# arghyasur1991/Spark-TTS

Hardware: AMD Instinct MI355X
Metric: audio samples/sec (whole node), Spark-TTS-0.5B greedy (higher is better)
Workload: dtype bf16 weights + KV, fp32 activations/accumulate (LLM); vocoder: fp32 operands split into 2 bf16 planes, 3 products on the bf16 matrix pipe, fp32 accumulate

## Files before the change

### spark-tts_amd/csrc/smi_llm.hip

```cpp
#include "smi_common.h"
#include <stdio.h>
#include <string.h>
#include <cmath>
#include <map>
#include <mutex>
#include <vector>

namespace {

constexpr int kMaxRows = SMI_MAX_ROWS;
constexpr int kHeadDim = 64;

struct RowDesc {
  int32_t slot, pos, token, flags;
};

struct SampRec {
  int32_t mode;
  int32_t top_k;
  float inv_temp, top_p;
  unsigned long long seed;
  int32_t has_seed, pad;
};

// ... 3247 lines not shown
  uint8_t slot_feat[kMaxRows];
  int lm_restrict;
  int seq_dirty[kMaxRows];
  SeqRec* seq;
  std::vector<SeqRec> hseq;
  int* tlist;
  std::vector<int32_t> host_tlist;
  float* lp;
  float* lp_part; float2* lp_rowc;
  uint16_t* phist;
  int64_t* poll_dev; int64_t* poll_host;
  int32_t* pen_idx; size_t pen_idx_cap;
  std::vector<int32_t> host_pen_idx;
  float* logits; int* tok;
  float* cand_v; int* cand_i; unsigned int* cand_n;
  unsigned long long* stamps; int stamps_on;
  int max_steps;
  int tune[4];
  int graph_steps;
  int pf_inline;
  int pf_qkv_eighths;
  int prefetch_mask, prefetch_rows;
  int tune2;
  int pgemm_min_rows;
  int pg_min[4];
  int wd_parts;
  int exact;
  int gu1_lo;
  int gu1_rows;
  hipGraphExec_t graph; uint64_t graph_id;
  std::map<hipGraphExec_t, hipStream_t> graph_last;
  std::map<uint64_t, hipGraphExec_t> graph_cache;
  hipEvent_t ev0, ev1;
  std::vector<RowDesc> host_rows;
#ifdef SMI_DIAG
  EngState eng;
  int eng_on;
#endif
};

namespace {

std::vector<const void*>& lds_big_kernels() {
  static std::vector<const void*> v;
  return v;
}
bool lds_big_register(const void* f) {
  lds_big_kernels().push_back(f);
  return true;
}
template <auto F>
struct LdsBig {
  static inline const bool reg = lds_big_register((const void*)F);
};
constexpr int kLdsBigBytes = 160 * 1024;

void pages_release(smi_llm* L, int slot) {
  for (int i = 0; i < L->slot_pages[slot]; ++i) {
    const int32_t pg = L->hptab[(size_t)slot * L->ppslot + i];
    if (--L->page_ref[pg] == 0) L->free_pages.push_back(pg);
  }
  L->slot_pages[slot] = 0;
}
void pages_share(smi_llm* L, int src, int dst, int n) {
  for (int i = 0; i < n; ++i) {
    const int32_t pg = L->hptab[(size_t)src * L->ppslot + i];
// ... 664 lines not shown

template <int PRO, int EPI, int NTW = 2, int WR = 1, int RING = 0, int XMAP = 0, int TWO = 0, int MTB = 8>
int launch_pgemm(const smi_llm* L, GemmP p, hipStream_t st, int nsplit = 1) {
  constexpr int cols = (4 / WR) * NTW;
  constexpr int rows = MTB * 16;
  const dim3 grid2((p.NT + cols - 1) / cols, (p.M + rows - 1) / rows);
  dim3 grid = XMAP ? dim3(grid2.x * grid2.y) : grid2;
  constexpr size_t lds = (RING ? (size_t)RING * (12 * rows + cols * 64) : (size_t)2 * 12 * rows) * 16 + (TWO ? 0 : rows * 4);
  if constexpr (lds > 64 * 1024) {
    static_cast<void>(LdsBig<k_pgemm<PRO, EPI, 1, NTW, WR, RING, XMAP, TWO, MTB>>::reg);
    static_cast<void>(LdsBig<k_pgemm<PRO, EPI, 0, NTW, WR, RING, XMAP, TWO, MTB>>::reg);
    static_assert(lds <= (size_t)kLdsBigBytes, "k_pgemm: LDS beyond the opted-in window");
  }
  const int mtiles = (p.M + 15) / 16;
  if (nsplit > 1) {
    SMI_REQUIRE(EPI == EPI_RESID && XMAP && RING >= 3 && p.kseg > 0 && nsplit <= 16, "launch_pgemm: split-K is the RESID ring form's");
    SMI_REQUIRE(L->pslab && (size_t)nsplit * p.NT * mtiles * 1024 <= L->pslab_bytes, "launch_pgemm: partial slab too small");
    p.slab = L->pslab; p.slab_mt = mtiles;
    grid = dim3(grid2.x * grid2.y, nsplit);
  }
  if (L->cfg.kv_dtype) hipLaunchKernelGGL((k_pgemm<PRO, EPI, 1, NTW, WR, RING, XMAP, TWO, MTB>), grid, dim3(256), lds, st, p);
  else hipLaunchKernelGGL((k_pgemm<PRO, EPI, 0, NTW, WR, RING, XMAP, TWO, MTB>), grid, dim3(256), lds, st, p);
  SMI_LAUNCH_CHECK();
  if (nsplit > 1) {
    DownCP d;
    d.W = nullptr; d.NT = p.NT; d.KT = p.KT; d.M = p.M; d.wperm = 0; d.XS = nullptr; d.part = L->pslab;
    d.Y = p.Y; d.Yin = p.Yin; d.gamma_next = p.gamma_next; d.XSout = p.XSout; d.ssout = p.ssout;
    hipLaunchKernelGGL((k_resid_comb<1, 1>), dim3(p.NT * mtiles), dim3(64), 0, st, d, nsplit, mtiles);
    SMI_LAUNCH_CHECK();
  }
  return SMI_OK;
}

int launch_layers_big(smi_llm* L, const RowDesc* rows, int M, int family, hipStream_t st) {
  const smi_llm_cfg& c = L->cfg;
  const bool pg = family == PF_PGEMM;
  const bool gq = L->pg_forced ? M < L->pg_min[0] : !pg, go = L->pg_forced ? M < L->pg_min[1] : !pg,
             gg = L->pg_forced ? M < L->pg_min[2] : !pg, gd = L->pg_forced ? M < L->pg_min[3] : !pg;
  const int np_from_d = gd ? L->NTh * 4 : L->NTh, np_from_o = go ? L->NTh * 4 : L->NTh;
  const bool few = M <= L->pg_split_rows && !(L->tune2 & 16384);
  const int kseg_o = (L->KTq + kPgSegO - 1) / kPgSegO, kseg_d = (L->KTi + kPgSegD - 1) / kPgSegD;
  const int nseg_o = (L->KTq + kseg_o - 1) / kseg_o, nseg_d = (L->KTi + kseg_d - 1) / kseg_d;
  int rc;
  for (int l = 0; l < c.num_layers; ++l) {
    const GemmP p = gemm_operands(L, KQKV, l, L->big, rows, M, np_from_d);
    if (gq) rc = launch_gemm<1, 16, 2, 1, PRO_NORM, EPI_QKV>(L, p, st);
    else if (L->tune2 & 16384) rc = launch_pgemm<PRO_NORM, EPI_QKV>(L, p, st);
    else if (few) rc = launch_pgemm<PRO_NORM, EPI_QKV, 2, 2, 6, 1, 0, 4>(L, p, st);
    else rc = launch_pgemm<PRO_NORM, EPI_QKV, 6, 2, 3, 1>(L, p, st);
    if (rc) return rc;
    if (l == c.num_layers - 1) break;
    const AttnP a = attn_operands(L, l, L->big, rows, M);
    if (L->tune2 & 1024) {
      if ((rc = c.kv_dtype ? launch_attn<1>(L, a, 0, st) : launch_attn<0>(L, a, 0, st))) return rc;
    } else {
      const dim3 ag((unsigned)((M + kAttnWaves - 1) / kAttnWaves), (unsigned)c.num_heads);
      if (!c.kv_dtype && L->attn_pf2 && L->pf_ntiles > 0 && c.head_dim == 64) {
        const int tasks = L->pf_ntiles * c.num_heads;
        hipLaunchKernelGGL(k_attn_pf2, dim3((tasks + 3) / 4), dim3(256), 0, st, a, (const PfTile*)L->pf_tiles, L->pf_ntiles);
      } else if (c.kv_dtype) hipLaunchKernelGGL((k_attn_pf<1>), ag, dim3(kAttnWaves * 64), 0, st, a);
      else hipLaunchKernelGGL((k_attn_pf<0>), ag, dim3(kAttnWaves * 64), 0, st, a);
      SMI_LAUNCH_CHECK();
    }
    GemmP o = gemm_operands(L, KO, l, L->big, rows, M, np_from_d);
    o.kseg = kseg_o;
    if (go) rc = launch_oproj(L, o, M, st);
    else if (L->tune2 & 16384) rc = launch_pgemm<PRO_PLAIN, EPI_RESID>(L, o, st);
    else if (few) rc = launch_pgemm<PRO_PLAIN, EPI_RESID, 2, 2, 6, 1, 0, 4>(L, o, st, nseg_o);
    else rc = launch_pgemm<PRO_PLAIN, EPI_RESID, 4, 2, 4, 1>(L, o, st);
    if (rc) return rc;
    const GemmP g = gemm_operands(L, KGU, l, L->big, rows, M, np_from_o);
    if (gg) rc = launch_gemm<1, 8, 4, 1, PRO_NORM, EPI_SWIGLU, 1, 2>(L, g, st);
    else if (L->tune2 & 512) rc = launch_pgemm<PRO_NORM, EPI_SWIGLU>(L, g, st);
    else if (L->tune2 & 16384) rc = launch_pgemm<PRO_NORM, EPI_SWIGLU, 4>(L, g, st);
    else if (L->tune2 & 32768) rc = launch_pgemm<PRO_NORM, EPI_SWIGLU, 8, 2, 3>(L, g, st);
    else if (few) rc = launch_pgemm<PRO_NORM, EPI_SWIGLU, 2, 2, 4, 0, 0, 4>(L, g, st);
    else rc = launch_pgemm<PRO_NORM, EPI_SWIGLU, 8, 2, 2, 0, 1>(L, g, st);
    if (rc) return rc;
    GemmP d = gemm_operands(L, KD, l, L->big, rows, M, np_from_o);
    d.wperm = L->wd_parts; d.kseg = kseg_d;
    if (gd) rc = launch_gemm<1, 16, 2, 5, PRO_PLAIN, EPI_RESID>(L, d, st);
    else if (L->tune2 & 16384) rc = launch_pgemm<PRO_PLAIN, EPI_RESID>(L, d, st);
    else if (few) rc = launch_pgemm<PRO_PLAIN, EPI_RESID, 2, 2, 6, 1, 0, 4>(L, d, st, nseg_d);
// ... 11 lines not shown
void work_free(Work& w) {
  void* ptrs[] = {w.h, w.q, w.xs_h, w.xs_attn, w.xs_act, w.ss};
  for (void* q : ptrs)
    if (q) (void)hipFree(q);
  w = Work{};
}

int ensure_big(smi_llm* L, int rows) {
  if (rows <= L->big_rows) return SMI_OK;
  work_free(L->big);
  L->big_rows = 0;
  if (L->pslab) (void)hipFree(L->pslab);
  L->pslab = nullptr; L->pslab_bytes = 0;
  {
    const size_t mt = ((size_t)(rows < kPgSplitRows ? rows : kPgSplitRows) + 15) / 16;
    const size_t bytes = (size_t)16 * L->NTh * mt * 1024;
    if (hipMalloc((void**)&L->pslab, bytes) != hipSuccess) { smi_set_error("hipMalloc(prefill split-K slab, %zu bytes) failed", bytes); return SMI_ENOMEM; }
    L->pslab_bytes = bytes;
  }
  if (!work_alloc(L, L->big, (size_t)rows)) { smi_set_error("hipMalloc(prefill workspace for %d rows) failed", rows); return SMI_ENOMEM; }
  L->big_rows = rows;
  return SMI_OK;
}

int launch_embed(smi_llm* L, const RowDesc* rows, int M, hipStream_t st) {
  hipLaunchKernelGGL(k_embed, dim3((M + 3) / 4), dim3(256), 0, st, (const uint16_t*)sec(L, SMI_LLM_LM_HEAD, 0), L->KTh, rows, M,
                     (const float*)sec(L, SMI_LLM_LN1, 0), L->dec.h, L->dec.xs_h, L->dec.ss, L->NTh * 4, L->exact);
  SMI_LAUNCH_CHECK();
  return SMI_OK;
}

int launch_layers(smi_llm* L, const RowDesc* rows, int M, bool kv_only_last, hipStream_t st) {
  int rc;
  for (int l = 0; l < L->cfg.num_layers; ++l) {
    if ((rc = launch_one(L, KQKV, l, rows, M, nullptr, st))) return rc;
    if (kv_only_last && l == L->cfg.num_layers - 1) break;
    if ((rc = launch_one(L, KATTN, l, rows, M, nullptr, st))) return rc;
    if ((rc = launch_one(L, KO, l, rows, M, nullptr, st))) return rc;
    if ((rc = launch_one(L, KGU, l, rows, M, nullptr, st))) return rc;
    if ((rc = launch_one(L, KD, l, rows, M, nullptr, st))) return rc;
  }
  return SMI_OK;
}

int launch_step(smi_llm* L, int M, hipStream_t st) {
  int rc;
  if (eng_usable(L, L->rows, M)) {
    if ((rc = eng_launch(L, st))) return rc;
  } else if ((rc = launch_layers(L, L->rows, M, false, st))) return rc;
  if ((rc = launch_one(L, KLM, 0, L->rows, M, nullptr, st))) return rc;
  return launch_one(L, KFIN, 0, L->rows, M, nullptr, st);
}

int ensure_plan(smi_llm* L, size_t rows) {
  if (rows <= L->plan_cap) return SMI_OK;
  if (L->plan) (void)hipFree(L->plan);
  L->plan = nullptr; L->plan_cap = 0;
  size_t cap = rows + 1024;
  if (hipMalloc((void**)&L->plan, cap * sizeof(RowDesc)) != hipSuccess) {
    smi_set_error("hipMalloc(prefill plan, %zu rows) failed", cap);
    return SMI_ENOMEM;
  }
  L->plan_cap = cap;
  return SMI_OK;
}

struct PollArgs {
  int32_t slot[kMaxRows];
  int32_t from[kMaxRows];
};
__global__ __launch_bounds__(64) void k_poll(const int64_t* hist, const int32_t* count, const int32_t* finished, int max_steps,
                                             PollArgs a, int cap, int64_t* stage) {
  const int i = blockIdx.x, sl = a.slot[i], from = a.from[i];
  int64_t* rec = stage + (size_t)i * (1 + cap);
  const int cnt = count[sl];
  if (threadIdx.x == 0) {
    int2 head; head.x = cnt; head.y = finished[sl];
    *(int2*)rec = head;
  }
  int end = cnt < max_steps ? cnt : max_steps;
  if (end - from > cap) end = from + cap;
  for (int t = from + (int)threadIdx.x; t < end; t += 64) rec[1 + (t - from)] = hist[(size_t)t * kMaxRows + sl];
}

// ... 171 lines not shown
      hipMemset(L->count, 0, kMaxRows * 4) != hipSuccess || hipMemset(L->finished, 0, kMaxRows * 4) != hipSuccess ||
      hipMemset(L->step, 0, 4) != hipSuccess) {
    smi_set_error("hipMemset of scratch failed");
    smi_llm_destroy(L);
    return SMI_EHIP;
  }
  if (hipFuncSetAttribute((const void*)k_lm32<7>, hipFuncAttributeMaxDynamicSharedMemorySize, 160 * 1024) != hipSuccess) (void)hipGetLastError();
  if (hipFuncSetAttribute((const void*)k_lm32<8>, hipFuncAttributeMaxDynamicSharedMemorySize, 160 * 1024) != hipSuccess) (void)hipGetLastError();
  if (hipFuncSetAttribute((const void*)k_lm32<7, 1>, hipFuncAttributeMaxDynamicSharedMemorySize, 160 * 1024) != hipSuccess) (void)hipGetLastError();
  if (hipFuncSetAttribute((const void*)k_lm32<8, 1>, hipFuncAttributeMaxDynamicSharedMemorySize, 160 * 1024) != hipSuccess) (void)hipGetLastError();
  {
    static std::mutex mu;
    static bool done[64] = {};
    int dev = 0;
    std::lock_guard<std::mutex> lk(mu);
    if (hipGetDevice(&dev) != hipSuccess || dev < 0 || dev >= 64) {
      smi_set_error("smi_llm_create: no current device");
      smi_llm_destroy(L);
      return SMI_EHIP;
    }
    for (size_t i = 0; i < lds_big_kernels().size() && !done[dev]; ++i)
      if (hipFuncSetAttribute(lds_big_kernels()[i], hipFuncAttributeMaxDynamicSharedMemorySize, kLdsBigBytes) != hipSuccess) {
        smi_set_error("smi_llm_create: hipFuncSetAttribute(MaxDynamicSharedMemorySize) failed: %s", hipGetErrorString(hipGetLastError()));
        smi_llm_destroy(L);
        return SMI_EHIP;
      }
    done[dev] = true;
  }
  if (hipEventCreate(&L->ev0) != hipSuccess || hipEventCreate(&L->ev1) != hipSuccess) {
    smi_set_error("hipEventCreate failed");
    smi_llm_destroy(L);
    return SMI_EHIP;
  }
#ifdef SMI_DIAG
  L->eng_on = 0;
  snprintf(L->eng.why, sizeof(L->eng.why), "off (opt-in: SPARKMI_ENGINE=1 or smi_llm_set_engine)");
  { const char* e = smi_env("SPARKMI_ENGINE");
    if (e && e[0] == '1') {
      const int rce = eng_create(L);
      if (rce) { smi_llm_destroy(L); return rce; }
      L->eng_on = L->eng.enabled;
    }
  }
#endif
  *out = L;
  return SMI_OK;
}

int smi_llm_destroy(smi_llm* L) {
  if (!L) return SMI_OK;
  graphs_flush(L);
  eng_destroy(L);
  work_free(L->dec);
  work_free(L->big);
  void* ptrs[] = {L->part_o, L->h2, L->dpart, L->fuse_cnt, L->rows, L->plan, L->pf_tiles, L->pval, L->pidx, L->hist,
                  L->count, L->finished, L->step, L->ctl, L->ptab, L->kcache, L->vcache, L->logits, L->tok, L->cand_v, L->cand_i, L->cand_n, L->stamps, L->pslab, L->apart,
                  L->phist, L->pen_idx, L->lp, L->lp_part, L->lp_rowc, L->tlist, L->poll_dev, L->seq};
  for (void* q : ptrs)
    if (q) (void)hipFree(q);
  if (L->poll_host) (void)hipHostFree(L->poll_host);
  if (L->ev0) (void)hipEventDestroy(L->ev0);
  if (L->ev1) (void)hipEventDestroy(L->ev1);
  delete L;
  return SMI_OK;
}

int smi_llm_set_sampling(smi_llm* L, int do_sample, float temperature, int top_k, float top_p, uint64_t seed) {
  SMI_REQUIRE(L, "smi_llm_set_sampling: null handle");
  if (do_sample) {
    SMI_REQUIRE(temperature > 0.f, "smi_llm_set_sampling: temperature must be > 0");
    SMI_REQUIRE(top_k >= 1 && top_k <= kSampleCap, "smi_llm_set_sampling: top_k must be in 1..%d", kSampleCap);
    SMI_REQUIRE(top_p > 0.f && top_p <= 1.f, "smi_llm_set_sampling: top_p must be in (0, 1]");
    if (top_k > L->cfg.vocab_size) top_k = L->cfg.vocab_size;
  }
  const bool changed = L->do_sample != (do_sample ? 1 : 0) ||
                       (do_sample && (L->temperature != temperature || L->top_k != top_k || L->top_p != top_p));
  L->do_sample = do_sample ? 1 : 0;
  L->temperature = temperature; L->top_k = top_k; L->top_p = top_p; L->seed = seed;
  L->hctl.seed = seed;
  SMI_HIP(hipMemcpy(&L->ctl->seed, &seed, sizeof(seed), hipMemcpyHostToDevice));
  if (changed) graphs_flush(L);
  return SMI_OK;
}

static int validate_prompts(const smi_llm* L, const int64_t* ids, const int32_t* lens, int B, int P_max) {
  for (int b = 0; b < B; ++b) {
    SMI_REQUIRE(lens[b] >= 1 && lens[b] <= P_max, "smi_llm_prefill: lens[%d]=%d outside 1..%d", b, lens[b], P_max);
    SMI_REQUIRE(lens[b] < L->cfg.max_positions, "smi_llm_prefill: prompt %d longer than max_positions", b);
    for (int t = 0; t < lens[b]; ++t) {
      const int64_t id = ids[(size_t)b * P_max + t];
      SMI_REQUIRE(id >= 0 && id < L->cfg.vocab_size, "smi_llm_prefill: token id %lld out of range", (long long)id);
    }
  }
  return SMI_OK;
}

static int prefill_prompts(smi_llm* L, const int64_t* ids, const int32_t* lens, int B, int P_max, const int32_t* slots,
                           size_t* tail_off, hipStream_t st, const int32_t* n_ret = nullptr, const int32_t* tail_slots = nullptr,
                           const std::vector<RowDesc>* extra = nullptr) {
  size_t total = 0;
  { const int rcv = validate_prompts(L, ids, lens, B, P_max); if (rcv) return rcv; }
  for (int b = 0; b < B; ++b) total += lens[b] - 1;
  {
    int longest = 0;
    for (int b = 0; b < B; ++b) longest = lens[b] > longest ? lens[b] : longest;
    L->attn_seg = segs_for(longest);
  }
  const bool chunks_only = smi_env("SPARKMI_PREFILL_CHUNKS") != nullptr || L->exact;
  auto cls_of = [&](int b) -> int {
    const int r = lens[b] - 1;
    if (chunks_only) return 0;
    if (L->pg_forced) return total > (size_t)kMaxRows ? 3 : 0;
    return r <= kMaxRows ? 0 : r < L->pf_long ? 1 : 2;
  };
  size_t ncls[4] = {0, 0, 0, 0};
  for (int b = 0; b < B; ++b) ncls[cls_of(b)] += lens[b] - 1;
  const size_t nchunks = (ncls[0] + kMaxRows - 1) / kMaxRows;
  const size_t off2 = 0, off1 = ncls[2], off3 = off1 + ncls[1], off0 = off3 + ncls[3], tail = off0 + nchunks * kMaxRows;
  int rc;
  const size_t nextra = extra ? extra->size() : 0;
  if ((rc = ensure_plan(L, tail + kMaxRows + nextra))) return rc;
  L->host_rows.assign(tail + kMaxRows + nextra, RowDesc{0, 0, 0, 0});
  {
    size_t w[4] = {off0, off1, off2, off3};
    for (int b = 0; b < B; ++b) {
      size_t& r = w[cls_of(b)];
      for (int t = 0; t + 1 < lens[b]; ++t) L->host_rows[r++] = RowDesc{slots[b], t, (int32_t)ids[(size_t)b * P_max + t], 0};
    }
  }
  for (int b = 0, j = 0; b < B; ++b)
    for (int r = 0; r < (n_ret ? n_ret[b] : 1); ++r, ++j)
      L->host_rows[tail + j] = RowDesc{tail_slots ? tail_slots[j] : slots[b], lens[b] - 1, (int32_t)ids[(size_t)b * P_max + lens[b] - 1], 0};
  for (size_t e = 0; e < nextra; ++e) L->host_rows[tail + kMaxRows + e] = (*extra)[e];
  SMI_HIP(hipMemcpyAsync(L->plan, L->host_rows.data(), L->host_rows.size() * sizeof(RowDesc), hipMemcpyHostToDevice, st));
  const size_t pass_off[3] = {off2, off1, off3}, pass_rows[3] = {ncls[2], ncls[1], ncls[3]};
  const int pass_family[3] = {PF_PGEMM, PF_GROUPED, PF_PGEMM};
  for (int ps = 0; ps < 3; ++ps) {
    if (pass_rows[ps] == 0) continue;
    constexpr size_t kBigRows = 4096;
    if ((rc = ensure_big(L, (int)(pass_rows[ps] < kBigRows ? pass_rows[ps] : kBigRows)))) return rc;
    for (size_t q0 = 0; q0 < pass_rows[ps]; q0 += kBigRows) {
      const size_t r0 = pass_off[ps] + q0;
      const int M = (int)((pass_rows[ps] - q0) < kBigRows ? (pass_rows[ps] - q0) : kBigRows);
      const RowDesc* rows = L->plan + r0;
      L->pf_ntiles = 0;
      if (!L->cfg.kv_dtype && L->attn_pf2) {
        std::vector<PfTile>& T = L->host_tiles;
        T.clear();
        for (int i = 0; i < M;) {
          const RowDesc& a0 = L->host_rows[r0 + i];
          int n = 1;
          while (n < 16 && i + n < M && L->host_rows[r0 + i + n].slot == a0.slot && L->host_rows[r0 + i + n].pos == a0.pos + n) ++n;
          T.push_back(PfTile{i, n, a0.slot, a0.pos});
          i += n;
        }
        if (T.size() > L->pf_tiles_cap) {
          if (L->pf_tiles) (void)hipFree(L->pf_tiles);
          L->pf_tiles = nullptr; L->pf_tiles_cap = 0;
          const size_t cap = T.size() + 256;
          if (hipMalloc((void**)&L->pf_tiles, cap * sizeof(PfTile)) != hipSuccess) { smi_set_error("hipMalloc(prefill attention tiles) failed"); return SMI_ENOMEM; }
          L->pf_tiles_cap = cap;
        }
        SMI_HIP(hipMemcpyAsync(L->pf_tiles, T.data(), T.size() * sizeof(PfTile), hipMemcpyHostToDevice, st));
        L->pf_ntiles = (int)T.size();
      }
      const bool d_grouped = L->pg_forced ? M < L->pg_min[3] : pass_family[ps] == PF_GROUPED;
      hipLaunchKernelGGL(k_embed, dim3((M + 3) / 4), dim3(256), 0, st, (const uint16_t*)sec(L, SMI_LLM_LM_HEAD, 0), L->KTh, rows, M,
                         (const float*)sec(L, SMI_LLM_LN1, 0), L->big.h, L->big.xs_h, L->big.ss, d_grouped ? L->NTh * 4 : L->NTh, 0);
      SMI_LAUNCH_CHECK();
      if ((rc = launch_layers_big(L, rows, M, pass_family[ps], st))) return rc;
    }
  }
  for (size_t c = 0; c < nchunks; ++c) {
    const int M = (int)((ncls[0] - c * kMaxRows) < (size_t)kMaxRows ? (ncls[0] - c * kMaxRows) : kMaxRows);
    const RowDesc* rows = L->plan + off0 + c * kMaxRows;
    if ((rc = launch_embed(L, rows, M, st))) return rc;
    if ((rc = launch_layers(L, rows, M, true, st))) return rc;
  }
  *tail_off = tail;
  return SMI_OK;
}

static void live_set(smi_llm* L, const int* slots, int n) {
  L->B = n;
  L->live_order.assign(slots, slots + n);
  L->identity_slots = 1;
  L->lm_restrict = n > 0;
  for (int b = 0; b < n; ++b) {
    L->identity_slots &= slots[b] == b;
    L->lm_restrict &= (L->slot_feat[slots[b]] & F_ALLOW) != 0;
  }
  L->graph = nullptr;
}

static int validate_eos(const int64_t* eos_ids, int n_eos) {
  SMI_REQUIRE(n_eos >= 0 && n_eos <= SMI_MAX_EOS && (n_eos == 0 || eos_ids), "eos list: 0..%d ids", SMI_MAX_EOS);
  return SMI_OK;
}

static int gen_reset(smi_llm* L, const int64_t* eos_ids, int n_eos, int nseq, hipStream_t st) {
  L->started = 0;
  for (int b = 0; b < kMaxRows; ++b) L->hctl.seqid[b] = nseq ? b : 0;
  slots_clear(L);
  L->admit_seq = nseq;
  if (L->paged)
    for (int b = 0; b < kMaxRows; ++b) pages_release(L, b);
  memset(L->slot_busy, 0, sizeof(L->slot_busy));
  memset(L->slot_len, 0, sizeof(L->slot_len));
  live_set(L, nullptr, 0);
  for (int e = 0; e < SMI_MAX_EOS; ++e) L->hctl.eos[e] = e < n_eos ? (long long)eos_ids[e] : -1;
  L->hctl.n_eos = n_eos;
  L->hctl.seed = L->seed;
  SMI_HIP(hipMemcpyAsync(L->ctl, &L->hctl, sizeof(Ctl), hipMemcpyHostToDevice, st));
  SMI_HIP(hipMemsetAsync(L->count, 0, kMaxRows * 4, st));
  SMI_HIP(hipMemsetAsync(L->finished, 0, kMaxRows * 4, st));
  SMI_HIP(hipMemsetAsync(L->step, 0, 4, st));
  L->session = nseq == 0;
  L->started = 1;
  return SMI_OK;
}

int smi_llm_prefill(smi_llm* L, const int64_t* ids, const int32_t* lens, int B, int P_max, const int64_t* eos_ids, int n_eos,
                    void* stream) {
  SMI_REQUIRE(L && ids && lens, "smi_llm_prefill: null argument");
  SMI_REQUIRE(B >= 1 && B <= L->cfg.max_slots, "smi_llm_prefill: B=%d outside 1..%d", B, L->cfg.max_slots);
  hipStream_t st = (hipStream_t)stream;
  int32_t slots[kMaxRows];
  for (int b = 0; b < kMaxRows; ++b) slots[b] = b;
  int rc;
  if ((rc = validate_prompts(L, ids, lens, B, P_max)) || (rc = validate_eos(eos_ids, n_eos))) return rc;
  if (L->paged) {
    long need = 0;
    for (int b = 0; b < B; ++b) need += (lens[b] + (1 << L->pshift) - 1) >> L->pshift;
    if (need > L->cfg.kv_pages) {
      smi_set_error("KV page pool too small for these prompts: %ld pages of %d tokens needed, the pool has %d", need, 1 << L->pshift, L->cfg.kv_pages);
      return SMI_ENOMEM;
    }
  }
  if ((rc = gen_reset(L, eos_ids, n_eos, B, st))) return rc;
  if ((rc = pages_ensure(L, slots, lens, B, st))) { L->started = 0; return rc; }
  for (int b = 0; b < B; ++b) { L->slot_busy[b] = 1; L->slot_len[b] = lens[b] + 1; }
  live_set(L, slots, B);
  size_t tail = 0;
  if ((rc = prefill_prompts(L, ids, lens, B, P_max, slots, &tail, st))) { L->started = 0; return rc; }
  if (hipMemcpyAsync(L->rows, L->plan + tail, kMaxRows * sizeof(RowDesc), hipMemcpyDeviceToDevice, st) != hipSuccess) {
    L->started = 0;
    smi_set_error("smi_llm_prefill: copying the first step's rows failed");
    return SMI_EHIP;
  }
  if ((rc = launch_embed(L, L->rows, B, st)) || (rc = launch_step(L, B, st))) { L->started = 0; return rc; }
  return SMI_OK;
}

int smi_llm_session_begin(smi_llm* L, const int64_t* eos_ids, int n_eos, void* stream) {
  SMI_REQUIRE(L, "smi_llm_session_begin: null handle");
  { const int rcv = validate_eos(eos_ids, n_eos); if (rcv) return rcv; }
  return gen_reset(L, eos_ids, n_eos, 0, (hipStream_t)stream);
}

static int session_set_rows(smi_llm* L, const std::vector<RowDesc>& live, hipStream_t st) {
  int slots[kMaxRows];
  for (size_t b = 0; b < live.size(); ++b) slots[b] = live[b].slot;
  live_set(L, slots, (int)live.size());
  if (L->B == 0) return SMI_OK;
  L->host_rows.assign(kMaxRows, RowDesc{0, 0, 0, 0});
  for (int b = 0; b < L->B; ++b) L->host_rows[b] = live[b];
  SMI_HIP(hipMemcpyAsync(L->rows, L->host_rows.data(), kMaxRows * sizeof(RowDesc), hipMemcpyHostToDevice, st));
  SMI_HIP(hipStreamSynchronize(st));
  return launch_embed(L, L->rows, L->B, st);
}

static int session_live_rows(smi_llm* L, std::vector<RowDesc>& live, hipStream_t st) {
  live.assign((size_t)L->B, RowDesc{0, 0, 0, 0});
  SMI_HIP(hipStreamSynchronize(st));
  if (L->B) SMI_HIP(hipMemcpy(live.data(), L->rows, (size_t)L->B * sizeof(RowDesc), hipMemcpyDeviceToHost));
  return SMI_OK;
}

static int validate_sampling(const smi_sample_params* sp, int n) {
  if (!sp) return SMI_OK;
  for (int b = 0; b < n; ++b) {
    const smi_sample_params& r = sp[b];
    SMI_REQUIRE(r.mode == SMI_SAMPLING_INHERIT || r.mode == SMI_SAMPLING_GREEDY || r.mode == SMI_SAMPLING_SAMPLE,
// ... 314 lines not shown
    if (L->paged)
      for (int j = 0; j < N; ++j) pages_release(L, slots[j]);
  };
  if (hipMemcpyAsync(L->ctl, &L->hctl, sizeof(Ctl), hipMemcpyHostToDevice, st) != hipSuccess) {
    undo();
    smi_set_error("smi_llm_admit: uploading the generation controls failed");
    return SMI_EHIP;
  }
  if ((rc = allow_tiles_upload(L, st))) { undo(); return rc; }
  for (int j = 0; j < N; ++j) {
    const int sl = slots[j];
    const SeqRec rec = seq_record(seq ? &seq[j] : nullptr, ids + (size_t)src[j] * P_max, lens_j[j]);
    const int on = rec.n_bias > 0 || rec.n_stop > 0;
    L->slot_feat[sl] |= (rec.n_bias > 0 ? F_BIAS : 0) | (rec.n_stop > 0 ? F_STOP : 0);
    if (!on && !L->seq_dirty[sl]) continue;
    L->hseq[(size_t)sl] = rec;
    L->seq_dirty[sl] = on;
    if (hipMemcpyAsync(L->seq + sl, &L->hseq[(size_t)sl], sizeof(SeqRec), hipMemcpyHostToDevice, st) != hipSuccess) {
      L->seq_dirty[sl] = 1;
      undo();
      smi_set_error("smi_llm_admit_biased: uploading the sequence records failed");
      return SMI_EHIP;
    }
  }
  std::vector<RowDesc> fork;
  int fork_span = 0;
  if (forked)
    for (int j = 0; j < N; ++j) {
      const int b = src[j], p0 = L->paged ? shared_pages(b) << L->pshift : 0, p1 = lens[b] - 1;
      if (slots[j] == lead[b] || p1 <= p0) continue;
      fork.push_back(RowDesc{lead[b], slots[j], p0, p1});
      fork_span = p1 - p0 > fork_span ? p1 - p0 : fork_span;
    }
  size_t tail = 0;
  if ((rc = prefill_prompts(L, ids, lens, n, P_max, lead, &tail, st, n_ret, slots, fork.empty() ? nullptr : &fork))) { undo(); return rc; }
  if (!fork.empty()) {
    ForkP fp;
    fp.work = (const int4*)(L->plan + tail + kMaxRows);
    fp.kcache = (unsigned char*)L->kcache; fp.vcache = (unsigned char*)L->vcache;
    fp.piece_shift = L->cfg.kv_dtype ? 4 : 3;
    fp.layer_bytes = L->kv_layer_elems * (L->cfg.kv_dtype ? 4 : 2);
    fp.n_kv = L->cfg.num_kv_heads; fp.max_pos = L->cfg.max_positions;
    fp.km = kv_map(L);
    const dim3 grid((unsigned)(((size_t)fork_span << fp.piece_shift) + 255) / 256, (unsigned)fork.size(),
                    (unsigned)(L->cfg.num_layers * 2 * L->cfg.num_kv_heads));
    hipLaunchKernelGGL(k_kv_fork, grid, dim3(256), 0, st, fp);
    SMI_LAUNCH_CHECK();
  }
  int32_t zeros[kMaxRows] = {0};
  for (int j = 0; j < N; ++j) {
    SMI_HIP(hipMemcpyAsync(L->count + slots[j], zeros, 4, hipMemcpyHostToDevice, st));
    SMI_HIP(hipMemcpyAsync(L->finished + slots[j], zeros, 4, hipMemcpyHostToDevice, st));
  }
  SMI_HIP(hipMemcpyAsync(L->rows, L->plan + tail, kMaxRows * sizeof(RowDesc), hipMemcpyDeviceToDevice, st));
  if (forked) {
    std::vector<int64_t> eids((size_t)N * P_max);
    for (int j = 0; j < N; ++j) memcpy(&eids[(size_t)j * P_max], ids + (size_t)src[j] * P_max, (size_t)P_max * 8);
    if ((rc = pen_histories(L, eids.data(), lens_j, N, P_max, slots, st))) return rc;
  } else if ((rc = pen_histories(L, ids, lens, n, P_max, slots, st))) {
    return rc;
  }
  const std::vector<int> before = L->live_order;
  live_set(L, slots, N);
  if ((rc = launch_embed(L, L->rows, N, st)) || (rc = launch_step(L, N, st))) {
    live_set(L, before.data(), (int)before.size());
    L->lm_restrict = 0;
    return rc;
  }
  std::vector<RowDesc> fresh;
  if ((rc = session_live_rows(L, fresh, st))) return rc;
  for (int j = 0; j < N; ++j) {
    live.push_back(fresh[j]);
    L->slot_busy[slots[j]] = 1;
    L->slot_len[slots[j]] = lens_j[j] + 1;
    slots_out[j] = slots[j];
  }
  return session_set_rows(L, live, st);
}

int smi_llm_admit(smi_llm* L, const int64_t* ids, const int32_t* lens, int n, int P_max, int32_t* slots_out, void* stream) {
  return admit(L, AdmitReq{ids, lens, n, P_max}, slots_out, (hipStream_t)stream);
}
int smi_llm_admit_sampled(smi_llm* L, const int64_t* ids, const int32_t* lens, int n, int P_max, const smi_sample_params* params,
                          int32_t* slots_out, void* stream) {
  return admit(L, AdmitReq{ids, lens, n, P_max, nullptr, params}, slots_out, (hipStream_t)stream);
}
int smi_llm_admit_penalized(smi_llm* L, const int64_t* ids, const int32_t* lens, int n, int P_max, const smi_sample_params* params,
                            const smi_penalty_params* pens, int32_t* slots_out, void* stream) {
  return admit(L, AdmitReq{ids, lens, n, P_max, nullptr, params, pens}, slots_out, (hipStream_t)stream);
}
int smi_llm_admit_logprobs(smi_llm* L, const int64_t* ids, const int32_t* lens, int n, int P_max, const smi_sample_params* params,
                           const smi_penalty_params* pens, const int32_t* want_lp, int32_t* slots_out, void* stream) {
  return admit(L, AdmitReq{ids, lens, n, P_max, nullptr, params, pens, want_lp}, slots_out, (hipStream_t)stream);
}
int smi_llm_admit_forked(smi_llm* L, const int64_t* ids, const int32_t* lens, int n, int P_max, const int32_t* n_ret,
                         const smi_sample_params* params, const smi_penalty_params* pens, const int32_t* want_lp, int32_t* slots_out,
                         void* stream) {
  return admit(L, AdmitReq{ids, lens, n, P_max, n_ret, params, pens, want_lp}, slots_out, (hipStream_t)stream);
}
int smi_llm_admit_constrained(smi_llm* L, const int64_t* ids, const int32_t* lens, int n, int P_max, const int32_t* n_ret,
                              const smi_sample_params* params, const smi_penalty_params* pens, const int32_t* want_lp,
// ... 493 lines not shown
}

int smi_llm_debug_hidden(smi_llm* L, float* out_host, int n) {
  SMI_REQUIRE(L && out_host && n >= L->H, "smi_llm_debug_hidden: out holds %d floats, %d needed", n, L ? L->H : 0);
  SMI_HIP(hipDeviceSynchronize());
  SMI_HIP(hipMemcpy(out_host, L->dec.h, (size_t)L->H * 4, hipMemcpyDeviceToHost));
  return eng_check(L);
}

int smi_llm_debug_read(smi_llm* L, int what, void* out_host, size_t cap, size_t* got) {
  SMI_REQUIRE(L && out_host && got, "smi_llm_debug_read: null argument");
  const void* src = nullptr;
  size_t n = 0;
  const size_t R = L->B > 0 ? (size_t)L->B : 1;
  switch (what) {
    case 0: src = L->dec.q; n = R * L->Q * 4; break;
    case 1: src = L->dec.xs_attn; n = R * L->Q * 6; break;
    case 2: src = L->dec.xs_act; n = R * L->I * 6; break;
    case 3: src = L->dec.xs_h; n = R * L->H * 6; break;
    case 4: src = L->dec.h; n = R * L->H * 4; break;
    case 5: src = L->eng.gran; n = L->eng.gran ? (size_t)2 * L->eng.gran_per_buf * 8 : 0; break;
    case 6: src = L->dec.ss; n = R * L->H; break;
    case 7: src = L->kcache; n = (size_t)L->cfg.max_positions * kHeadDim * 2; break;
    case 8: src = L->h2; n = (size_t)L->H * 4; break;
    default: smi_set_error("smi_llm_debug_read: what=%d", what); return SMI_EINVAL;
  }
  SMI_REQUIRE(src && n <= cap, "smi_llm_debug_read: buffer %d holds %zu bytes, out holds %zu", what, n, cap);
  SMI_HIP(hipDeviceSynchronize());
  SMI_HIP(hipMemcpy(out_host, src, n, hipMemcpyDeviceToHost));
  *got = n;
  return SMI_OK;
}

static int debug_kv_check(const smi_llm* L, int layer, int slot, int pos0, int n) {
  SMI_REQUIRE(L && !L->paged, "debug KV access needs a contiguous KV cache (kv_page_tokens = 0)");
  SMI_REQUIRE(layer >= 0 && layer < L->cfg.num_layers && slot >= 0 && slot < L->cfg.max_slots && pos0 >= 0 && n >= 0 &&
              pos0 + n <= L->cfg.max_positions, "debug KV access: layer %d slot %d positions %d..%d out of range", layer, slot, pos0, pos0 + n);
  return SMI_OK;
}

int smi_llm_debug_set_kv(smi_llm* L, int layer, int slot, int pos0, int n, const float* k_host, const float* v_host) {
  { const int rc = debug_kv_check(L, layer, slot, pos0, n); if (rc) return rc; }
  SMI_REQUIRE(k_host && v_host, "smi_llm_debug_set_kv: null argument");
  SMI_HIP(hipDeviceSynchronize());
  const int nkv = L->cfg.num_kv_heads, f32 = L->cfg.kv_dtype;
  const size_t esz = f32 ? 4 : 2;
  std::vector<unsigned char> buf((size_t)n * kHeadDim * esz);
  for (int isv = 0; isv < 2; ++isv)
    for (int kh = 0; kh < nkv; ++kh) {
      for (int t = 0; t < n; ++t)
        for (int i = 0; i < kHeadDim; ++i) {
          const int d = isv ? i : (i >> 1) + 32 * (i & 1);
          const float x = (isv ? v_host : k_host)[((size_t)t * nkv + kh) * kHeadDim + d];
          if (f32) ((float*)buf.data())[(size_t)t * kHeadDim + i] = x;
          else {
            uint32_t u; memcpy(&u, &x, 4);
            ((uint16_t*)buf.data())[(size_t)t * kHeadDim + i] = (uint16_t)((u + 0x7FFFu + ((u >> 16) & 1u)) >> 16);
          }
        }
      unsigned char* base = (unsigned char*)kv_layer(L, isv ? L->vcache : L->kcache, layer);
      const size_t row0 = ((size_t)slot * nkv + kh) * L->cfg.max_positions + pos0;
      SMI_HIP(hipMemcpy(base + row0 * kHeadDim * esz, buf.data(), buf.size(), hipMemcpyHostToDevice));
    }
  return SMI_OK;
}

int smi_llm_debug_get_kv(smi_llm* L, int layer, int slot, int pos0, int n, float* k_host, float* v_host) {
  { const int rc = debug_kv_check(L, layer, slot, pos0, n); if (rc) return rc; }
  SMI_REQUIRE(k_host && v_host, "smi_llm_debug_get_kv: null argument");
  SMI_HIP(hipDeviceSynchronize());
  const int nkv = L->cfg.num_kv_heads, f32 = L->cfg.kv_dtype;
  const size_t esz = f32 ? 4 : 2;
  std::vector<unsigned char> buf((size_t)n * kHeadDim * esz);
  for (int isv = 0; isv < 2; ++isv)
    for (int kh = 0; kh < nkv; ++kh) {
      const unsigned char* base = (const unsigned char*)kv_layer(L, isv ? L->vcache : L->kcache, layer);
      const size_t row0 = ((size_t)slot * nkv + kh) * L->cfg.max_positions + pos0;
      SMI_HIP(hipMemcpy(buf.data(), base + row0 * kHeadDim * esz, buf.size(), hipMemcpyDeviceToHost));
      for (int t = 0; t < n; ++t)
        for (int i = 0; i < kHeadDim; ++i) {
          const int d = isv ? i : (i >> 1) + 32 * (i & 1);
          float x;
          if (f32) x = ((const float*)buf.data())[(size_t)t * kHeadDim + i];
          else { const uint32_t u = (uint32_t)((const uint16_t*)buf.data())[(size_t)t * kHeadDim + i] << 16; memcpy(&x, &u, 4); }
          (isv ? v_host : k_host)[((size_t)t * nkv + kh) * kHeadDim + d] = x;
        }
    }
  return SMI_OK;
}

int smi_llm_debug_layer(smi_llm* L, int layer, int M, const int32_t* rows_host, const float* hidden_host, int stage) {
  SMI_REQUIRE(L && rows_host && hidden_host && M >= 1 && M <= kMaxRows, "smi_llm_debug_layer: bad argument");
  SMI_REQUIRE(layer >= 0 && layer < L->cfg.num_layers && stage >= 0 && stage <= 4, "smi_llm_debug_layer: layer %d stage %d", layer, stage);
  SMI_REQUIRE(!L->paged, "smi_llm_debug_layer needs a contiguous KV cache");
  SMI_HIP(hipDeviceSynchronize());
  graphs_flush(L);
  std::vector<RowDesc> rows(kMaxRows, RowDesc{0, 0, 0, 0});
  int maxpos = 0, ident = 1;
  for (int m = 0; m < M; ++m) {
    const int sl = rows_host[2 * m], ps = rows_host[2 * m + 1];
    SMI_REQUIRE(sl >= 0 && sl < L->cfg.max_slots && ps >= 0 && ps < L->cfg.max_positions, "smi_llm_debug_layer: row %d = (slot %d, pos %d)", m, sl, ps);
    rows[m] = RowDesc{sl, ps, 0, 0};
    maxpos = ps > maxpos ? ps : maxpos;
    ident &= sl == m;
  }
  SMI_HIP(hipMemcpy(L->rows, rows.data(), rows.size() * sizeof(RowDesc), hipMemcpyHostToDevice));
  L->B = M; L->identity_slots = ident; L->session = 0; L->started = 0;
  L->attn_seg = segs_for(maxpos + 1);
  float* src = nullptr;
  SMI_HIP(hipMalloc((void**)&src, (size_t)M * L->H * 4));
  int rc = SMI_OK;
// ... 247 lines not shown
```

Before: 564,500.

## Overlap first decode step's layers with last prefill pass on a side stream

Adds a second non-blocking stream and per-layer events so the first generation step's per-layer work runs on a tail stream. Each tail layer is gated on the matching layer of the last big prefill pass via an event, instead of waiting for the whole prefill to finish. Small-chunk prefill is moved ahead of the big passes when overlapping, and admit_forked is reordered so its setup copies happen before the prefill run. This should hide the decode step's latency behind prefill, at the cost of more complexity, extra event overhead and contention for compute units. It also extends debug KV reads to paged caches.

```diff
diff --git a/spark-tts_amd/csrc/smi_llm.hip b/spark-tts_amd/csrc/smi_llm.hip
--- a/spark-tts_amd/csrc/smi_llm.hip
+++ b/spark-tts_amd/csrc/smi_llm.hip
@@ -3303,6 +3303,9 @@
   std::map<hipGraphExec_t, hipStream_t> graph_last;
   std::map<uint64_t, hipGraphExec_t> graph_cache;
   hipEvent_t ev0, ev1;
+  hipStream_t tail_st;
+  std::vector<hipEvent_t> tail_ev;
+  int pf_overlap;
   std::vector<RowDesc> host_rows;
 #ifdef SMI_DIAG
   EngState eng;
@@ -4033,7 +4036,23 @@
   return SMI_OK;
 }
 
-int launch_layers_big(smi_llm* L, const RowDesc* rows, int M, int family, hipStream_t st) {
+int launch_layer(smi_llm* L, int l, const RowDesc* rows, int M, bool kv_only_last, hipStream_t st) {
+  int rc;
+  if ((rc = launch_one(L, KQKV, l, rows, M, nullptr, st))) return rc;
+  if (kv_only_last && l == L->cfg.num_layers - 1) return SMI_OK;
+  if ((rc = launch_one(L, KATTN, l, rows, M, nullptr, st))) return rc;
+  if ((rc = launch_one(L, KO, l, rows, M, nullptr, st))) return rc;
+  if ((rc = launch_one(L, KGU, l, rows, M, nullptr, st))) return rc;
+  return launch_one(L, KD, l, rows, M, nullptr, st);
+}
+
+int tail_layer(smi_llm* L, int l, int tailM, hipStream_t st) {
+  SMI_HIP(hipEventRecord(L->tail_ev[(size_t)l], st));
+  SMI_HIP(hipStreamWaitEvent(L->tail_st, L->tail_ev[(size_t)l], 0));
+  return launch_layer(L, l, L->rows, tailM, false, L->tail_st);
+}
+
+int launch_layers_big(smi_llm* L, const RowDesc* rows, int M, int family, hipStream_t st, int tailM = 0) {
   const smi_llm_cfg& c = L->cfg;
   const bool pg = family == PF_PGEMM;
   const bool gq = L->pg_forced ? M < L->pg_min[0] : !pg, go = L->pg_forced ? M < L->pg_min[1] : !pg,
@@ -4050,6 +4069,7 @@
     else if (few) rc = launch_pgemm<PRO_NORM, EPI_QKV, 2, 2, 6, 1, 0, 4>(L, p, st);
     else rc = launch_pgemm<PRO_NORM, EPI_QKV, 6, 2, 3, 1>(L, p, st);
     if (rc) return rc;
+    if (tailM && (rc = tail_layer(L, l, tailM, st))) return rc;
     if (l == c.num_layers - 1) break;
     const AttnP a = attn_operands(L, l, L->big, rows, M);
     if (L->tune2 & 1024) {
@@ -4127,24 +4147,24 @@
 
 int launch_layers(smi_llm* L, const RowDesc* rows, int M, bool kv_only_last, hipStream_t st) {
   int rc;
-  for (int l = 0; l < L->cfg.num_layers; ++l) {
-    if ((rc = launch_one(L, KQKV, l, rows, M, nullptr, st))) return rc;
-    if (kv_only_last && l == L->cfg.num_layers - 1) break;
-    if ((rc = launch_one(L, KATTN, l, rows, M, nullptr, st))) return rc;
-    if ((rc = launch_one(L, KO, l, rows, M, nullptr, st))) return rc;
-    if ((rc = launch_one(L, KGU, l, rows, M, nullptr, st))) return rc;
-    if ((rc = launch_one(L, KD, l, rows, M, nullptr, st))) return rc;
-  }
+  for (int l = 0; l < L->cfg.num_layers; ++l)
+    if ((rc = launch_layer(L, l, rows, M, kv_only_last, st))) return rc;
   return SMI_OK;
 }
 
+int launch_step_layers(smi_llm* L, int M, hipStream_t st) {
+  if (eng_usable(L, L->rows, M)) return eng_launch(L, st);
+  return launch_layers(L, L->rows, M, false, st);
+}
+int launch_step_head(smi_llm* L, int M, hipStream_t st) {
+  int rc;
+  if ((rc = launch_one(L, KLM, 0, L->rows, M, nullptr, st))) return rc;
+  return launch_one(L, KFIN, 0, L->rows, M, nullptr, st);
+}
 int launch_step(smi_llm* L, int M, hipStream_t st) {
   int rc;
-  if (eng_usable(L, L->rows, M)) {
-    if ((rc = eng_launch(L, st))) return rc;
-  } else if ((rc = launch_layers(L, L->rows, M, false, st))) return rc;
-  if ((rc = launch_one(L, KLM, 0, L->rows, M, nullptr, st))) return rc;
-  return launch_one(L, KFIN, 0, L->rows, M, nullptr, st);
+  if ((rc = launch_step_layers(L, M, st))) return rc;
+  return launch_step_head(L, M, st);
 }
 
 int ensure_plan(smi_llm* L, size_t rows) {
@@ -4382,6 +4402,15 @@
     smi_llm_destroy(L);
     return SMI_EHIP;
   }
+  L->pf_overlap = !smi_env("SPARKMI_PREFILL_SERIAL");
+  L->tail_ev.assign((size_t)cfg->num_layers + 2, nullptr);
+  bool tail_ok = hipStreamCreateWithFlags(&L->tail_st, hipStreamNonBlocking) == hipSuccess;
+  for (hipEvent_t& e : L->tail_ev) tail_ok = tail_ok && hipEventCreateWithFlags(&e, hipEventDisableTiming) == hipSuccess;
+  if (!tail_ok) {
+    smi_set_error("smi_llm_create: creating the prefill tail stream / events failed");
+    smi_llm_destroy(L);
+    return SMI_EHIP;
+  }
 #ifdef SMI_DIAG
   L->eng_on = 0;
   snprintf(L->eng.why, sizeof(L->eng.why), "off (opt-in: SPARKMI_ENGINE=1 or smi_llm_set_engine)");
@@ -4401,6 +4430,9 @@
   if (!L) return SMI_OK;
   graphs_flush(L);
   eng_destroy(L);
+  if (L->tail_st) { (void)hipStreamSynchronize(L->tail_st); (void)hipStreamDestroy(L->tail_st); }
+  for (hipEvent_t e : L->tail_ev)
+    if (e) (void)hipEventDestroy(e);
   work_free(L->dec);
   work_free(L->big);
   void* ptrs[] = {L->part_o, L->h2, L->dpart, L->fuse_cnt, L->rows, L->plan, L->pf_tiles, L->pval, L->pidx, L->hist,
@@ -4445,9 +4477,14 @@
   return SMI_OK;
 }
 
-static int prefill_prompts(smi_llm* L, const int64_t* ids, const int32_t* lens, int B, int P_max, const int32_t* slots,
-                           size_t* tail_off, hipStream_t st, const int32_t* n_ret = nullptr, const int32_t* tail_slots = nullptr,
-                           const std::vector<RowDesc>* extra = nullptr) {
+struct PromptPlan {
+  size_t off[4], ncls[4];
+  size_t nchunks, tail;
+};
+
+static int prefill_plan(smi_llm* L, const int64_t* ids, const int32_t* lens, int B, int P_max, const int32_t* slots,
+                        PromptPlan* pp, hipStream_t st, const int32_t* n_ret = nullptr, const int32_t* tail_slots = nullptr,
+                        const std::vector<RowDesc>* extra = nullptr) {
   size_t total = 0;
   { const int rcv = validate_prompts(L, ids, lens, B, P_max); if (rcv) return rcv; }
   for (int b = 0; b < B; ++b) total += lens[b] - 1;
@@ -4483,8 +4520,46 @@
       L->host_rows[tail + j] = RowDesc{tail_slots ? tail_slots[j] : slots[b], lens[b] - 1, (int32_t)ids[(size_t)b * P_max + lens[b] - 1], 0};
   for (size_t e = 0; e < nextra; ++e) L->host_rows[tail + kMaxRows + e] = (*extra)[e];
   SMI_HIP(hipMemcpyAsync(L->plan, L->host_rows.data(), L->host_rows.size() * sizeof(RowDesc), hipMemcpyHostToDevice, st));
-  const size_t pass_off[3] = {off2, off1, off3}, pass_rows[3] = {ncls[2], ncls[1], ncls[3]};
+  const size_t offs[4] = {off0, off1, off2, off3};
+  for (int k = 0; k < 4; ++k) { pp->off[k] = offs[k]; pp->ncls[k] = ncls[k]; }
+  pp->nchunks = nchunks; pp->tail = tail;
+  return SMI_OK;
+}
+
+static int tail_join(smi_llm* L, hipStream_t st) {
+  hipEvent_t join = L->tail_ev.back();
+  SMI_HIP(hipEventRecord(join, L->tail_st));
+  SMI_HIP(hipStreamWaitEvent(st, join, 0));
+  return SMI_OK;
+}
+
+static int prefill_run(smi_llm* L, const PromptPlan& pp, int tailM, hipStream_t st) {
+  int rc;
+  const size_t* ncls = pp.ncls;
+  const size_t off0 = pp.off[0], nchunks = pp.nchunks;
+  const size_t pass_off[3] = {pp.off[2], pp.off[1], pp.off[3]}, pass_rows[3] = {ncls[2], ncls[1], ncls[3]};
   const int pass_family[3] = {PF_PGEMM, PF_GROUPED, PF_PGEMM};
+  int last_ps = -1;
+  for (int ps = 0; ps < 3; ++ps)
+    if (pass_rows[ps]) last_ps = ps;
+  bool overlap = tailM > 0 && L->pf_overlap && last_ps >= 0 && pass_family[last_ps] == PF_PGEMM && !L->pg_forced && !L->stamps_on &&
+                 !(L->tune2 & 1024) && !eng_usable(L, L->rows, tailM);
+  if (overlap) {
+    hipStreamCaptureStatus cs = hipStreamCaptureStatusNone;
+    if (hipStreamIsCapturing(st, &cs) != hipSuccess) { (void)hipGetLastError(); overlap = false; }
+    else overlap = cs == hipStreamCaptureStatusNone;
+  }
+  auto run_chunks = [&]() -> int {
+    for (size_t c = 0; c < nchunks; ++c) {
+      const int M = (int)((ncls[0] - c * kMaxRows) < (size_t)kMaxRows ? (ncls[0] - c * kMaxRows) : kMaxRows);
+      const RowDesc* rows = L->plan + off0 + c * kMaxRows;
+      int rcc;
+      if ((rcc = launch_embed(L, rows, M, st))) return rcc;
+      if ((rcc = launch_layers(L, rows, M, true, st))) return rcc;
+    }
+    return SMI_OK;
+  };
+  if (overlap && (rc = run_chunks())) return rc;
   for (int ps = 0; ps < 3; ++ps) {
     if (pass_rows[ps] == 0) continue;
     constexpr size_t kBigRows = 4096;
@@ -4518,17 +4593,22 @@
       hipLaunchKernelGGL(k_embed, dim3((M + 3) / 4), dim3(256), 0, st, (const uint16_t*)sec(L, SMI_LLM_LM_HEAD, 0), L->KTh, rows, M,
                          (const float*)sec(L, SMI_LLM_LN1, 0), L->big.h, L->big.xs_h, L->big.ss, d_grouped ? L->NTh * 4 : L->NTh, 0);
       SMI_LAUNCH_CHECK();
-      if ((rc = launch_layers_big(L, rows, M, pass_family[ps], st))) return rc;
-    }
-  }
-  for (size_t c = 0; c < nchunks; ++c) {
-    const int M = (int)((ncls[0] - c * kMaxRows) < (size_t)kMaxRows ? (ncls[0] - c * kMaxRows) : kMaxRows);
-    const RowDesc* rows = L->plan + off0 + c * kMaxRows;
-    if ((rc = launch_embed(L, rows, M, st))) return rc;
-    if ((rc = launch_layers(L, rows, M, true, st))) return rc;
-  }
-  *tail_off = tail;
-  return SMI_OK;
+      if (overlap && ps == last_ps && q0 + kBigRows >= pass_rows[ps]) {
+        hipEvent_t fork = L->tail_ev[(size_t)L->cfg.num_layers];
+        SMI_HIP(hipEventRecord(fork, st));
+        SMI_HIP(hipStreamWaitEvent(L->tail_st, fork, 0));
+        rc = launch_embed(L, L->rows, tailM, L->tail_st);
+        if (!rc) rc = launch_layers_big(L, rows, M, pass_family[ps], st, tailM);
+        const int rcj = tail_join(L, st);
+        if (rc || rcj) return rc ? rc : rcj;
+      } else if ((rc = launch_layers_big(L, rows, M, pass_family[ps], st))) return rc;
+    }
+  }
+  if (overlap) return SMI_OK;
+  if ((rc = run_chunks())) return rc;
+  if (tailM == 0) return SMI_OK;
+  if ((rc = launch_embed(L, L->rows, tailM, st))) return rc;
+  return launch_step_layers(L, tailM, st);
 }
 
 static void live_set(smi_llm* L, const int* slots, int n) {
@@ -4591,14 +4671,14 @@
   if ((rc = pages_ensure(L, slots, lens, B, st))) { L->started = 0; return rc; }
   for (int b = 0; b < B; ++b) { L->slot_busy[b] = 1; L->slot_len[b] = lens[b] + 1; }
   live_set(L, slots, B);
-  size_t tail = 0;
-  if ((rc = prefill_prompts(L, ids, lens, B, P_max, slots, &tail, st))) { L->started = 0; return rc; }
-  if (hipMemcpyAsync(L->rows, L->plan + tail, kMaxRows * sizeof(RowDesc), hipMemcpyDeviceToDevice, st) != hipSuccess) {
+  PromptPlan pp;
+  if ((rc = prefill_plan(L, ids, lens, B, P_max, slots, &pp, st))) { L->started = 0; return rc; }
+  if (hipMemcpyAsync(L->rows, L->plan + pp.tail, kMaxRows * sizeof(RowDesc), hipMemcpyDeviceToDevice, st) != hipSuccess) {
     L->started = 0;
     smi_set_error("smi_llm_prefill: copying the first step's rows failed");
     return SMI_EHIP;
   }
-  if ((rc = launch_embed(L, L->rows, B, st)) || (rc = launch_step(L, B, st))) { L->started = 0; return rc; }
+  if ((rc = prefill_run(L, pp, B, st)) || (rc = launch_step_head(L, B, st))) { L->started = 0; return rc; }
   return SMI_OK;
 }
 
@@ -4979,8 +5059,30 @@
       fork.push_back(RowDesc{lead[b], slots[j], p0, p1});
       fork_span = p1 - p0 > fork_span ? p1 - p0 : fork_span;
     }
-  size_t tail = 0;
-  if ((rc = prefill_prompts(L, ids, lens, n, P_max, lead, &tail, st, n_ret, slots, fork.empty() ? nullptr : &fork))) { undo(); return rc; }
+  PromptPlan pp;
+  if ((rc = prefill_plan(L, ids, lens, n, P_max, lead, &pp, st, n_ret, slots, fork.empty() ? nullptr : &fork))) { undo(); return rc; }
+  const size_t tail = pp.tail;
+  int32_t zeros[kMaxRows] = {0};
+  for (int j = 0; j < N; ++j) {
+    SMI_HIP(hipMemcpyAsync(L->count + slots[j], zeros, 4, hipMemcpyHostToDevice, st));
+    SMI_HIP(hipMemcpyAsync(L->finished + slots[j], zeros, 4, hipMemcpyHostToDevice, st));
+  }
+  SMI_HIP(hipMemcpyAsync(L->rows, L->plan + tail, kMaxRows * sizeof(RowDesc), hipMemcpyDeviceToDevice, st));
+  if (forked) {
+    std::vector<int64_t> eids((size_t)N * P_max);
+    for (int j = 0; j < N; ++j) memcpy(&eids[(size_t)j * P_max], ids + (size_t)src[j] * P_max, (size_t)P_max * 8);
+    if ((rc = pen_histories(L, eids.data(), lens_j, N, P_max, slots, st))) { undo(); return rc; }
+  } else if ((rc = pen_histories(L, ids, lens, n, P_max, slots, st))) {
+    undo();
+    return rc;
+  }
+  const std::vector<int> before = L->live_order;
+  live_set(L, slots, N);
+  auto unlive = [&]() {
+    live_set(L, before.data(), (int)before.size());
+    L->lm_restrict = 0;
+  };
+  if ((rc = prefill_run(L, pp, fork.empty() ? N : 0, st))) { unlive(); undo(); return rc; }
   if (!fork.empty()) {
     ForkP fp;
     fp.work = (const int4*)(L->plan + tail + kMaxRows);
@@ -4992,28 +5094,10 @@
     const dim3 grid((unsigned)(((size_t)fork_span << fp.piece_shift) + 255) / 256, (unsigned)fork.size(),
                     (unsigned)(L->cfg.num_layers * 2 * L->cfg.num_kv_heads));
     hipLaunchKernelGGL(k_kv_fork, grid, dim3(256), 0, st, fp);
-    SMI_LAUNCH_CHECK();
-  }
-  int32_t zeros[kMaxRows] = {0};
-  for (int j = 0; j < N; ++j) {
-    SMI_HIP(hipMemcpyAsync(L->count + slots[j], zeros, 4, hipMemcpyHostToDevice, st));
-    SMI_HIP(hipMemcpyAsync(L->finished + slots[j], zeros, 4, hipMemcpyHostToDevice, st));
-  }
-  SMI_HIP(hipMemcpyAsync(L->rows, L->plan + tail, kMaxRows * sizeof(RowDesc), hipMemcpyDeviceToDevice, st));
-  if (forked) {
-    std::vector<int64_t> eids((size_t)N * P_max);
-    for (int j = 0; j < N; ++j) memcpy(&eids[(size_t)j * P_max], ids + (size_t)src[j] * P_max, (size_t)P_max * 8);
-    if ((rc = pen_histories(L, eids.data(), lens_j, N, P_max, slots, st))) return rc;
-  } else if ((rc = pen_histories(L, ids, lens, n, P_max, slots, st))) {
-    return rc;
-  }
-  const std::vector<int> before = L->live_order;
-  live_set(L, slots, N);
-  if ((rc = launch_embed(L, L->rows, N, st)) || (rc = launch_step(L, N, st))) {
-    live_set(L, before.data(), (int)before.size());
-    L->lm_restrict = 0;
-    return rc;
-  }
+    if (hipGetLastError() != hipSuccess) { unlive(); smi_set_error("smi_llm_admit_forked: the fork copy's launch failed"); return SMI_EHIP; }
+    if ((rc = launch_embed(L, L->rows, N, st)) || (rc = launch_step_layers(L, N, st))) { unlive(); return rc; }
+  }
+  if ((rc = launch_step_head(L, N, st))) { unlive(); return rc; }
   std::vector<RowDesc> fresh;
   if ((rc = session_live_rows(L, fresh, st))) return rc;
   for (int j = 0; j < N; ++j) {
@@ -5573,8 +5657,8 @@
   return SMI_OK;
 }
 
-static int debug_kv_check(const smi_llm* L, int layer, int slot, int pos0, int n) {
-  SMI_REQUIRE(L && !L->paged, "debug KV access needs a contiguous KV cache (kv_page_tokens = 0)");
+static int debug_kv_check(const smi_llm* L, int layer, int slot, int pos0, int n, bool paged_ok = false) {
+  SMI_REQUIRE(L && (paged_ok || !L->paged), "debug KV writes need a contiguous KV cache (kv_page_tokens = 0)");
   SMI_REQUIRE(layer >= 0 && layer < L->cfg.num_layers && slot >= 0 && slot < L->cfg.max_slots && pos0 >= 0 && n >= 0 &&
               pos0 + n <= L->cfg.max_positions, "debug KV access: layer %d slot %d positions %d..%d out of range", layer, slot, pos0, pos0 + n);
   return SMI_OK;
@@ -5607,8 +5691,10 @@
 }
 
 int smi_llm_debug_get_kv(smi_llm* L, int layer, int slot, int pos0, int n, float* k_host, float* v_host) {
-  { const int rc = debug_kv_check(L, layer, slot, pos0, n); if (rc) return rc; }
+  { const int rc = debug_kv_check(L, layer, slot, pos0, n, true); if (rc) return rc; }
   SMI_REQUIRE(k_host && v_host, "smi_llm_debug_get_kv: null argument");
+  SMI_REQUIRE(!L->paged || ((pos0 + n + (1 << L->pshift) - 1) >> L->pshift) <= L->slot_pages[slot],
+              "smi_llm_debug_get_kv: slot %d holds no pages for positions %d..%d", slot, pos0, pos0 + n);
   SMI_HIP(hipDeviceSynchronize());
   const int nkv = L->cfg.num_kv_heads, f32 = L->cfg.kv_dtype;
   const size_t esz = f32 ? 4 : 2;
@@ -5616,8 +5702,16 @@
   for (int isv = 0; isv < 2; ++isv)
     for (int kh = 0; kh < nkv; ++kh) {
       const unsigned char* base = (const unsigned char*)kv_layer(L, isv ? L->vcache : L->kcache, layer);
-      const size_t row0 = ((size_t)slot * nkv + kh) * L->cfg.max_positions + pos0;
-      SMI_HIP(hipMemcpy(buf.data(), base + row0 * kHeadDim * esz, buf.size(), hipMemcpyDeviceToHost));
+      if (L->paged) {
+        for (int t = 0; t < n; ++t) {
+          const int pos = pos0 + t, pg = L->hptab[(size_t)slot * L->ppslot + (pos >> L->pshift)];
+          const size_t row = (((size_t)pg * nkv + kh) << L->pshift) + (size_t)(pos & ((1 << L->pshift) - 1));
+          SMI_HIP(hipMemcpy(buf.data() + (size_t)t * kHeadDim * esz, base + row * kHeadDim * esz, kHeadDim * esz, hipMemcpyDeviceToHost));
+        }
+      } else {
+        const size_t row0 = ((size_t)slot * nkv + kh) * L->cfg.max_positions + pos0;
+        SMI_HIP(hipMemcpy(buf.data(), base + row0 * kHeadDim * esz, buf.size(), hipMemcpyDeviceToHost));
+      }
       for (int t = 0; t < n; ++t)
         for (int i = 0; i < kHeadDim; ++i) {
           const int d = isv ? i : (i >> 1) + 32 * (i & 1);
```

Result: no change. 565,400 (median of 3 runs) (+0.2%).
